# DeadAt0m/LSQFakeQuantize-PyTorch

Measured on AMD Instinct MI355X. Metric: GElem/s fake-quant fwd+bwd, per-tensor int8, 1/2/4/8 MI355X; % HBM roofline, higher is better.
Workload: dtype f32

## Files before the change

lsqfakequantize-pytorch_amd/csrc/lsq_relayout.hip:

```cpp
#include <hip/hip_runtime.h>
#include <stdint.h>

#include "lsq_kernels.hpp"

namespace lsq {

constexpr int kRelTile = 64;

template <typename W>
__global__ __launch_bounds__(kBlock) void relayout_kernel(const W* __restrict__ src, W* __restrict__ dst, int64_t B, int64_t C,
                                                          int64_t tiles_b, int64_t tiles_c, int64_t tiles) {
    constexpr int TB = kRelTile;
    constexpr int kPerLane = TB * kRelTile / kBlock;
    __shared__ W tile[TB][kRelTile + 1];
    const int tid = static_cast<int>(threadIdx.x), lane = tid & 63, row0 = tid >> 6;
    const bool flat_r = C <= kRelTile, flat_w = B <= TB;
    const int nc_all = static_cast<int>(C < kRelTile ? C : kRelTile), nb_all = static_cast<int>(B < TB ? B : TB);
    int rq[kPerLane], wq[kPerLane];
    {
        const int q = kBlock / nc_all, r = kBlock - q * nc_all;
        int b = tid / nc_all, c = tid - b * nc_all;
#pragma unroll
        for (int k = 0; k < kPerLane; ++k) {
            rq[k] = (b << 8) | c;
            b += q; c += r;
            if (c >= nc_all) { c -= nc_all; ++b; }
        }
        const int q2 = kBlock / nb_all, r2 = kBlock - q2 * nb_all;
        int cc = tid / nb_all, bb = tid - cc * nb_all;
#pragma unroll
        for (int k = 0; k < kPerLane; ++k) {
            wq[k] = (bb << 8) | cc;
            cc += q2; bb += r2;
            if (bb >= nb_all) { bb -= nb_all; ++cc; }
        }
    }
    struct Where { const W* s; W* d; int nb, nc; };
    auto where = [&](int64_t t) {
        const int64_t tc = t % tiles_c, tb = (t / tiles_c) % tiles_b, a = t / (tiles_c * tiles_b);
        const int64_t b0 = tb * TB, c0 = tc * kRelTile;
        Where w;
        w.nb = static_cast<int>(B - b0 < TB ? B - b0 : TB);
        w.nc = static_cast<int>(C - c0 < kRelTile ? C - c0 : kRelTile);
        w.s = src + (a * B + b0) * C + c0;
        w.d = dst + (a * C + c0) * B + b0;
        return w;
    };
    W regs[kPerLane];
    auto fetch = [&](const Where& w) {
        if (flat_r) {
            const int n = w.nb * w.nc;
#pragma unroll
            for (int k = 0; k < kPerLane; ++k) {
                const int i = tid + k * kBlock;
                regs[k] = i < n ? w.s[i] : W(0);
            }
        } else {
#pragma unroll
            for (int k = 0; k < kPerLane; ++k) {
                const int b = row0 + k * (kBlock / 64);
                regs[k] = (b < w.nb && lane < w.nc) ? w.s[static_cast<int64_t>(b) * C + lane] : W(0);
            }
        }
    };
    int64_t t = blockIdx.x;
    if (t >= tiles) return;
    Where cur = where(t);
    fetch(cur);
    for (;;) {
        if (flat_r) {
            const int n = cur.nb * cur.nc;
#pragma unroll
            for (int k = 0; k < kPerLane; ++k)
                if (tid + k * kBlock < n) tile[rq[k] >> 8][rq[k] & 255] = regs[k];
        } else {
#pragma unroll
            for (int k = 0; k < kPerLane; ++k) tile[row0 + k * (kBlock / 64)][lane] = regs[k];
        }
        __syncthreads();
        const int64_t tn = t + gridDim.x;
        const bool more = tn < tiles;
        Where nxt = cur;
        if (more) {
            nxt = where(tn);
            fetch(nxt);
        }
        if (flat_w) {
            const int n = cur.nb * cur.nc;
#pragma unroll
            for (int k = 0; k < kPerLane; ++k) {
                const int i = tid + k * kBlock;
                if (i < n) cur.d[i] = tile[wq[k] >> 8][wq[k] & 255];
            }
        } else {
#pragma unroll
            for (int k = 0; k < kRelTile / (kBlock / 64); ++k) {
                const int c = row0 + k * (kBlock / 64);
                if (c < cur.nc && lane < cur.nb) cur.d[static_cast<int64_t>(c) * B + lane] = tile[lane][c];
            }
        }
        if (!more) break;
        __syncthreads();
        t = tn;
        cur = nxt;
    }
}

template <typename W>
static hipError_t launch_relayout(const void* src, void* dst, int64_t A, int64_t B, int64_t C, hipStream_t stream) {
    constexpr int TB = kRelTile;
    const int64_t tiles_b = (B + TB - 1) / TB, tiles_c = (C + kRelTile - 1) / kRelTile;
    const int64_t tiles = A * tiles_b * tiles_c;
    if (tiles <= 0) return hipSuccess;
    const int64_t resident = static_cast<int64_t>(device_info().cu_count) * 8;
    const dim3 grid(static_cast<unsigned>(tiles < resident ? tiles : resident));
    hipLaunchKernelGGL((relayout_kernel<W>), grid, dim3(kBlock), 0, stream, static_cast<const W*>(src), static_cast<W*>(dst), B, C,
                       tiles_b, tiles_c, tiles);
    return hipGetLastError();
}

hipError_t relayout(int elem_bytes, const void* src, void* dst, int64_t A, int64_t B, int64_t C, hipStream_t stream) {
    switch (elem_bytes) {
        case 2: return launch_relayout<uint16_t>(src, dst, A, B, C, stream);
        case 4: return launch_relayout<uint32_t>(src, dst, A, B, C, stream);
        case 8: return launch_relayout<uint64_t>(src, dst, A, B, C, stream);
        default: return hipErrorInvalidValue;
    }
}

}
```

Baseline: 306.1.

## Add vectorized 16-byte packet relayout kernel for 2-byte elements

```diff
diff --git a/lsqfakequantize-pytorch_amd/csrc/lsq_relayout.hip b/lsqfakequantize-pytorch_amd/csrc/lsq_relayout.hip
--- a/lsqfakequantize-pytorch_amd/csrc/lsq_relayout.hip
+++ b/lsqfakequantize-pytorch_amd/csrc/lsq_relayout.hip
@@ -2,6 +2,7 @@
 #include <stdint.h>
 
 #include "lsq_kernels.hpp"
+#include "lsq_relayout_geom.hpp"
 
 namespace lsq {
 
@@ -119,9 +120,104 @@
     return hipGetLastError();
 }
 
+typedef __attribute__((ext_vector_type(4))) unsigned int RelPacket;
+typedef RelPacket RelPacketAt2 __attribute__((aligned(2)));
+
+template <bool FLAT_R, bool FLAT_W>
+__global__ __launch_bounds__(rel16::kLanes) void relayout16_kernel(const uint16_t* __restrict__ src, uint16_t* __restrict__ dst,
+                                                                   const rel16::Geom launch_geom) {
+    using namespace rel16;
+    Geom g = launch_geom;
+    g.flat_r = FLAT_R;
+    g.flat_w = FLAT_W;
+    g.TC = tile_tc(FLAT_R, FLAT_W);
+    g.TB = kTileElems / g.TC;
+    __shared__ __attribute__((aligned(16))) uint16_t image[kTileElems];
+    auto lane_id = [] {
+        int tid = static_cast<int>(threadIdx.x);
+        asm volatile("" : "+v"(tid));
+        return tid;
+    };
+    RelPacket regs[kSlots];
+    auto fetch = [&](const Tile& T) {
+        const int tid = lane_id();
+#pragma unroll
+        for (int k = 0; k < kSlots; ++k) {
+            const Slot s = read_slot(g, T, tid, k);
+            if (s.n == kPacket) regs[k] = *reinterpret_cast<const RelPacketAt2*>(src + T.src0 + s.off);
+        }
+    };
+    int64_t t = blockIdx.x;
+    if (t >= g.tiles) return;
+    Tile cur = tile(g, t);
+    fetch(cur);
+    for (;;) {
+        int tid = lane_id();
+#pragma unroll
+        for (int k = 0; k < kSlots; ++k) {
+            const Slot s = read_slot(g, cur, tid, k);
+            if (s.n == kPacket) *reinterpret_cast<RelPacket*>(&image[lds_index(g, s.b, s.c)]) = regs[k];
+        }
+        if (ragged_reads(g, cur)) {
+#pragma unroll 1
+            for (int k = 0; k < kSlots; ++k) {
+                const Slot s = read_slot(g, cur, tid, k);
+                if (s.n < kPacket)
+                    for (int j = 0; j < s.n; ++j) image[lds_index(g, s.b, s.c) + j] = src[cur.src0 + s.off + j];
+            }
+        }
+        __syncthreads();
+        const int64_t tn = t + gridDim.x;
+        const bool more = tn < g.tiles;
+        Tile nxt = cur;
+        if (more) {
+            nxt = tile(g, tn);
+            fetch(nxt);
+        }
+        tid = lane_id();
+#pragma unroll 1
+        for (int k = 0; k < kSlots; ++k) {
+            const Slot s = write_slot(g, cur, tid, k);
+            uint16_t* p = dst + cur.dst0 + s.off;
+            int b = s.b, c = s.c;
+            if (s.n == kPacket) {
+                uint16_t e[kPacket];
+#pragma unroll
+                for (int j = 0; j < kPacket; ++j) {
+                    e[j] = image[lds_index(g, b, c)];
+                    write_step(g, cur, b, c);
+                }
+                RelPacket out;
+                __builtin_memcpy(&out, e, sizeof(RelPacket));
+                *reinterpret_cast<RelPacketAt2*>(p) = out;
+            } else {
+                for (int j = 0; j < s.n; ++j) {
+                    p[j] = image[lds_index(g, b, c)];
+                    write_step(g, cur, b, c);
+                }
+            }
+        }
+        if (!more) break;
+        __syncthreads();
+        t = tn;
+        cur = nxt;
+    }
+}
+
+static hipError_t launch_relayout16(const void* src, void* dst, int64_t A, int64_t B, int64_t C, hipStream_t stream) {
+    const rel16::Geom g = rel16::geom(A, B, C);
+    if (g.tiles <= 0) return hipSuccess;
+    const int64_t resident = static_cast<int64_t>(device_info().cu_count) * 8;
+    const dim3 grid(static_cast<unsigned>(g.tiles < resident ? g.tiles : resident));
+    auto* kernel = g.flat_r ? (g.flat_w ? relayout16_kernel<true, true> : relayout16_kernel<true, false>)
+                            : (g.flat_w ? relayout16_kernel<false, true> : relayout16_kernel<false, false>);
+    hipLaunchKernelGGL(kernel, grid, dim3(rel16::kLanes), 0, stream, static_cast<const uint16_t*>(src), static_cast<uint16_t*>(dst), g);
+    return hipGetLastError();
+}
+
 hipError_t relayout(int elem_bytes, const void* src, void* dst, int64_t A, int64_t B, int64_t C, hipStream_t stream) {
     switch (elem_bytes) {
-        case 2: return launch_relayout<uint16_t>(src, dst, A, B, C, stream);
+        case 2: return launch_relayout16(src, dst, A, B, C, stream);
         case 4: return launch_relayout<uint32_t>(src, dst, A, B, C, stream);
         case 8: return launch_relayout<uint64_t>(src, dst, A, B, C, stream);
         default: return hipErrorInvalidValue;
diff --git a/lsqfakequantize-pytorch_amd/csrc/lsq_relayout_geom.hpp b/lsqfakequantize-pytorch_amd/csrc/lsq_relayout_geom.hpp
--- /dev/null
+++ b/lsqfakequantize-pytorch_amd/csrc/lsq_relayout_geom.hpp
@@ -0,0 +1,119 @@
+#pragma once
+#include <stdint.h>
+
+#if defined(__HIPCC__)
+#define LSQ_REL_HD __host__ __device__ inline
+#else
+#define LSQ_REL_HD inline
+#endif
+
+namespace lsq {
+namespace rel16 {
+
+constexpr int kLanes = 256;
+constexpr int kPacket = 8;
+constexpr int kSlots = 4;
+constexpr int kTileElems = kLanes * kPacket * kSlots;
+constexpr int kFlatMax = 64;
+constexpr int kRunLanes = 8;
+
+struct Geom {
+    int64_t B, C, tiles_b, tiles_c, tiles;
+    int TB, TC;
+    int flat_r, flat_w;
+};
+
+struct Tile {
+    int64_t src0, dst0;
+    int nb, nc;
+};
+
+struct Slot {
+    int64_t off;
+    int n;
+    int b, c;
+};
+
+LSQ_REL_HD int tile_tc(bool flat_r, bool flat_w) { return (flat_w && !flat_r) ? kTileElems / kFlatMax : kFlatMax; }
+
+LSQ_REL_HD Geom geom(int64_t A, int64_t B, int64_t C) {
+    Geom g;
+    g.B = B;
+    g.C = C;
+    g.flat_r = C <= kFlatMax;
+    g.flat_w = B <= kFlatMax;
+    g.TC = tile_tc(g.flat_r, g.flat_w);
+    g.TB = kTileElems / g.TC;
+    g.tiles_b = (B + g.TB - 1) / g.TB;
+    g.tiles_c = (C + g.TC - 1) / g.TC;
+    g.tiles = A * g.tiles_b * g.tiles_c;
+    return g;
+}
+
+LSQ_REL_HD Tile tile(const Geom& g, int64_t t) {
+    const int64_t tc = t % g.tiles_c, tb = (t / g.tiles_c) % g.tiles_b, a = t / (g.tiles_c * g.tiles_b);
+    const int64_t b0 = tb * g.TB, c0 = tc * g.TC;
+    Tile T;
+    T.nb = static_cast<int>(g.B - b0 < g.TB ? g.B - b0 : g.TB);
+    T.nc = static_cast<int>(g.C - c0 < g.TC ? g.C - c0 : g.TC);
+    T.src0 = (a * g.B + b0) * g.C + c0;
+    T.dst0 = (a * g.C + c0) * g.B + b0;
+    return T;
+}
+
+LSQ_REL_HD int clamp_packet(int left) { return left < 0 ? 0 : (left > kPacket ? kPacket : left); }
+
+LSQ_REL_HD int lds_index(const Geom& g, int b, int c) {
+    if (g.flat_r) return b * static_cast<int>(g.C) + c;
+    return b * g.TC + ((c + kPacket * ((b >> 3) & 7)) & (g.TC - 1));
+}
+
+LSQ_REL_HD Slot read_slot(const Geom& g, const Tile& T, int lane, int k) {
+    const int p = lane + k * kLanes;
+    Slot s;
+    if (g.flat_r) {
+        const int e = p * kPacket;
+        s.off = e;
+        s.n = clamp_packet(T.nb * T.nc - e);
+        s.b = 0;
+        s.c = e;
+    } else {
+        const int per_row = g.TC / kPacket;
+        s.b = p / per_row;
+        s.c = (p % per_row) * kPacket;
+        s.off = static_cast<int64_t>(s.b) * g.C + s.c;
+        s.n = s.b < T.nb ? clamp_packet(T.nc - s.c) : 0;
+    }
+    return s;
+}
+
+LSQ_REL_HD bool ragged_reads(const Geom& g, const Tile& T) { return ((g.flat_r ? T.nb * T.nc : T.nc) % kPacket) != 0; }
+
+LSQ_REL_HD Slot write_slot(const Geom& g, const Tile& T, int lane, int k) {
+    Slot s;
+    if (g.flat_w) {
+        const int e = (lane + k * kLanes) * kPacket;
+        s.off = e;
+        s.n = clamp_packet(T.nb * T.nc - e);
+        s.c = e / T.nb;
+        s.b = e - s.c * T.nb;
+    } else {
+        const int blocks = g.TB / kPacket / kRunLanes;
+        s.b = ((lane % kRunLanes) + kRunLanes * (k % blocks)) * kPacket;
+        s.c = lane / kRunLanes + (kLanes / kRunLanes) * (k / blocks);
+        s.off = static_cast<int64_t>(s.c) * g.B + s.b;
+        s.n = s.c < T.nc ? clamp_packet(T.nb - s.b) : 0;
+    }
+    return s;
+}
+
+LSQ_REL_HD void write_step(const Geom& g, const Tile& T, int& b, int& c) {
+    ++b;
+    if (g.flat_w && b == T.nb) {
+        b = 0;
+        ++c;
+    }
+}
+
+}
+}
```

After: 301.3. 1.5% lower.
